# suhrig/arriba

Measured on AMD Instinct MI355X. Metric: chimeric reads/s end-to-end (BAM->fusions.tsv), synthetic, higher is better.
Workload: dtype int32

## Files before the change

### arriba_amd/_capi.py

```python
import ctypes
import os
from ctypes import POINTER, c_char_p, c_float, c_int, c_int32, c_size_t, c_uint8, c_uint16, c_uint32, c_uint64, c_void_p

LIB_DIR = os.path.join(os.path.dirname(os.path.abspath(__file__)), "lib")
FILTER_COUNT = 38
KERNEL_NAME_LENGTH = 48
FILTER_NAMES = [
    "", "duplicates", "inconsistently_clipped", "homopolymer", "read_through", "same_gene", "small_insert_size", "long_gap", "hairpin",
    "multimappers", "mismatches", "mismappers", "relative_support", "intronic", "non_coding_neighbors", "intragenic_exonic",
    "internal_tandem_duplication", "min_support", "known_fusions", "spliced", "blacklist", "end_to_end", "in_vitro", "merge_adjacent",
    "select_best", "marginal_read_through", "short_anchor", "no_coverage", "many_spliced", "no_genomic_support", "uninteresting_contigs",
    "viral_contigs", "top_expressed_viral_contigs", "low_coverage_viral_contigs", "genomic_support", "isoforms", "low_entropy", "homologs",
]


class FlatIndex(ctypes.Structure):
    _fields_ = [("n_contigs", c_uint32), ("contig_offset", POINTER(c_uint32)), ("n_keys", c_uint32), ("keys", POINTER(c_int32)),
                ("member_offset", POINTER(c_uint32)), ("n_members", c_uint32), ("members", POINTER(c_uint32))]


class AnnotationView(ctypes.Structure):
    _fields_ = [("n_genes", c_uint32), ("gene_contig", POINTER(c_uint16)), ("gene_start", POINTER(c_int32)), ("gene_end", POINTER(c_int32)),
                ("gene_bits", POINTER(c_uint8)), ("gene_exonic_length", POINTER(c_int32)),
                ("n_exons", c_uint32), ("exon_start", POINTER(c_int32)), ("exon_end", POINTER(c_int32)), ("exon_gene", POINTER(c_uint32)),
# ... 157 lines not shown
        "select_most_supported_breakpoints": (c_int, [ctx, POINTER(c_uint64)]),
        "recover_many_spliced": (c_int, [ctx, c_uint32, POINTER(c_uint64)]),
        "filter_in_vitro": (c_int, [ctx, c_float, POINTER(c_uint64)]),
        "filter_homologs": (c_int, [ctx, c_float, POINTER(c_uint64)]),
        "recover_isoforms": (c_int, [ctx, POINTER(c_uint64)]),
        "mark_genomic_support": (c_int, [ctx, POINTER(GenomicBreakpoint), c_uint32, c_int32, POINTER(c_uint64)]),
        "get_genomic_support": (c_int, [ctx, c_void_p, c_void_p]),
        "filter_no_genomic_support": (c_int, [ctx, POINTER(c_uint64)]),
        "recover_genomic_support": (c_int, [ctx, POINTER(c_uint64)]),
        "filter_blacklisted_ranges": (c_int, [ctx, POINTER(RangeRule), c_uint32, c_float, c_int32, POINTER(c_uint64)]),
        "recover_known_fusions": (c_int, [ctx, POINTER(RangeRule), c_uint32, c_int32, POINTER(c_uint64)]),
        "assign_confidence": (c_int, [ctx, c_void_p]),
        "recover_both_spliced": (c_int, [ctx, c_uint32, c_float, c_int32, c_uint32, POINTER(c_uint64)]),
        "set_owned_candidates": (c_int, [ctx, c_void_p, c_uint64]),
        "copy_multimapper_flags": (c_int, [ctx, c_void_p]),
        "multimappers_begin": (c_int, [ctx, c_void_p, POINTER(c_uint64)]),
        "multimappers_partial_best": (c_int, [ctx, c_void_p]),
        "multimappers_resolve": (c_int, [ctx, c_void_p, c_void_p, POINTER(c_uint64)]),
        "multimappers_recount": (c_int, [ctx, c_void_p, c_void_p]),
        "multimappers_finish": (c_int, [ctx, c_void_p, POINTER(c_uint64)]),
        "set_candidate_state": (c_int, [ctx, c_void_p, c_void_p, c_void_p, c_void_p]),
        "estimate_expected_fusions": (c_int, [ctx, c_uint64, c_void_p]),
        "get_evalues": (c_int, [ctx, c_void_p]),
        "filter_candidate_predicates": (c_int, [ctx, c_void_p]),
        "filter_relative_support": (c_int, [ctx, POINTER(c_uint64)]),
        "host_alloc": (c_void_p, [c_size_t]),
        "host_free": (None, [c_void_p]),
        "ingest_begin": (c_int, [ctx, POINTER(IngestConfig)]),
        "ingest_push": (c_int, [ctx, c_void_p, c_size_t]),
        "ingest_push_bgzf": (c_int, [ctx, c_void_p, c_size_t, POINTER(BgzfBlock), c_uint32, c_size_t]),
        "ingest_sam_targets": (c_int, [ctx, c_void_p, c_void_p, c_uint32]),
        "ingest_push_sam": (c_int, [ctx, c_void_p, c_size_t, c_uint64]),
        "sam_transcode": (c_int, [ctx, c_void_p, c_size_t, c_void_p, c_void_p, c_uint32, c_void_p, c_size_t, POINTER(c_uint64), POINTER(c_uint64), POINTER(c_uint64)]),
        "ingest_finish": (c_int, [ctx, POINTER(IngestResult)]),
        "shard_export_size": (c_int, [ctx, POINTER(c_uint64)]),
        "shard_export": (c_int, [ctx, c_void_p, c_uint64]),
        "shard_merge": (c_int, [ctx, c_void_p, c_uint64, c_uint32, POINTER(IngestResult)]),
        "mismapper_jobs": (c_int, [ctx, POINTER(c_uint64)]),
        "mismapper_verdicts": (c_int, [ctx, c_int32, c_uint32, c_uint32, c_void_p]),
        "filter_mismappers_apply": (c_int, [ctx, c_void_p, POINTER(c_uint64), POINTER(c_uint64)]),
        "get_viral_read_counts": (c_int, [ctx, c_void_p]),
        "get_coverage": (c_int, [ctx, c_void_p, c_void_p, c_void_p]),
        "detect_strandedness": (c_int, [ctx, POINTER(c_int)]),
        "get_read_lengths": (c_int, [ctx, c_uint64, c_uint64, c_void_p, c_void_p]),
        "gather_rows_begin": (c_int, [ctx, c_void_p, c_uint64, POINTER(c_uint64), POINTER(c_uint64), POINTER(c_uint64)]),
        "gather_rows_copy": (c_int, [ctx, POINTER(BatchRows)]),
        "set_profiling": (c_int, [ctx, c_int]),
        "debug_fail_allocation_in_finish": (None, [c_int]),
        "keep_batch_buffers": (c_int, [ctx, c_int]),
        "get_kernel_profile": (c_int, [ctx, c_void_p, c_void_p, c_void_p, c_uint32, POINTER(c_uint32)]),
        "last_kernel_ms": (c_int, [ctx, POINTER(c_float)]),
        "last_kernel_bytes": (c_int, [ctx, POINTER(c_uint64)]),
    }
    for name, (restype, argtypes) in signatures.items():
        function = getattr(lib, prefix + name, None)
        if function is None:
            continue
        function.restype = restype
        function.argtypes = argtypes
        setattr(api, name, function)
    api.exported = sorted(name for name in signatures if hasattr(api, name))
    api.declared = sorted(signatures)
    return api


def bind_host_api(lib):
# ... 132 lines not shown
```

### arriba_amd/csrc/device/agpu_ingest.hip

```cpp
#include <hip/hip_runtime.h>
#include <algorithm>
#include <cstring>
#include <string>
#include <vector>
#include <rocprim/rocprim.hpp>
#include "agpu_context.hpp"
#include "ingest_core.hpp"
#include "device_utils.hpp"
#include "shard_host.hpp"
#include "crc32_core.hpp"
#include "inflate_fast_core.hpp"

using namespace agpu;
namespace agpu { extern thread_local bool g_inside_ingest_finish; }

namespace {

const int BLOCK = 256;
inline unsigned int grid_for(uint64_t n, int block = BLOCK) { return (unsigned int) ((n + block - 1) / block); }

enum { IC_ACTIVE = 0, IC_MAPPED_READS = 1, IC_MISSING_HI = 2, IC_BROKEN = 3, IC_MALFORMED = 4, IC_CHIMERIC = 5, IC_COLLISION = 6, IC_MISMATCH = 7, IC_UNSORTED = 8, IC_MAX_NAME = 9,
       IC_MAX_READ_LENGTH = 10, IC_STRAND_COUNT = 11, IC_STRAND_MATCHING = 12, IC_RUNS_UNSORTED = 13, IC_QNAME_COMMA = 14, IC_COUNT = 16 };

#define HIP_CHECK(call) do { hipError_t e_ = (call); if (e_ != hipSuccess) { set_last_error(std::string(#call) + ": " + hipGetErrorString(e_)); return AGPU_ERR_DEVICE; } } while (0)
// ... 329 lines not shown
	const FragmentSizes mine = sizes[ref];
	cigar_words[i] = mine.cigar_words; sequence_bytes[i] = mine.sequence_bytes; name_lengths[i] = mine.name_length;
	uint32_t differs = 0;
	if (i > 0 && qname_run != nullptr) differs = qname_run[ref >> 1] != qname_run[order[i - 1] >> 1];
	else if (i > 0) {
		const Rec a = load_record(in, group_first[ref >> 1]), b = load_record(in, group_first[order[i - 1] >> 1]);
		const uint32_t length = qname_length(a);
		differs = length != qname_length(b);
		for (uint32_t k = 0; k < length && !differs; ++k) differs = a.name[k] != b.name[k];
	}
	new_group[i] = differs;
}

__global__ void __launch_bounds__(BLOCK) AGPU_PACK_OCCUPANCY fragment_pack_kernel(IngestStream in, const uint32_t* group_first, const uint32_t* order, uint64_t n, const FragmentPlan* plain, const TandemPlan* itd,
                                                              const uint64_t* cigar_base, const uint64_t* sequence_base, const uint64_t* name_base, const uint32_t* group_id, PackTarget out, uint32_t* counters) {
	__shared__ uint32_t block_max;
	if (threadIdx.x == 0) block_max = 0;
	__syncthreads();
	const uint64_t i = blockIdx.x * (uint64_t) BLOCK + threadIdx.x;
	if (i == n) out.name_offset[n] = name_base[n];
	if (i < n) {
		const uint32_t ref = order[i], g = ref >> 1;
		const bool is_itd = ref & 1;
		Fragment3 f;
		normalize_plan(in, is_itd ? itd[g].plan : plain[g], is_itd ? &itd[g].tandem : nullptr, f);
		Rec storage;
		const FragmentName name = name_of(in, group_first, ref, storage);
		atomicMax(&block_max, write_fragment(in, f, name, i, cigar_base[i], sequence_base[i], name_base[i], group_id[i], out));
	}
	__syncthreads();
	if (threadIdx.x == 0 && block_max) atomicMax(&counters[IC_MAX_READ_LENGTH], block_max);
}

template <bool INFLATED> __global__ void __launch_bounds__(256) bgzf_crc_kernel(const uint8_t* raw, const agpu_bgzf_block* blocks, uint32_t n_blocks, const Crc32Tables* tables, unsigned int* mismatches) {
	__shared__ uint32_t slice[4][256];
	__shared__ uint32_t join[2][4][256];
	__shared__ uint32_t staged[4][CRC32_WAVE_LANES * (CRC32_ROUND_WORDS + 1)];
	for (uint32_t k = threadIdx.x; k < 4 * 256; k += 256) ((uint32_t*) slice)[k] = ((const uint32_t*) tables->slice)[k];
	for (uint32_t k = threadIdx.x; k < 2 * 4 * 256; k += 256) ((uint32_t*) join)[k] = ((const uint32_t*) tables->join)[k];
	const uint32_t wave = threadIdx.x / CRC32_WAVE_LANES, lane = threadIdx.x % CRC32_WAVE_LANES, b = blockIdx.x * 4 + wave;
	agpu_bgzf_block block;
	block.crc32 = 0; block.payload_size = 0; block.raw_offset = 0; block.payload_offset = 0;
	if (b < n_blocks) block = blocks[b];
	if (INFLATED) { block.raw_offset = block.stream_offset; block.payload_offset = 0; block.payload_size = block.isize; }
	const bool checked = b < n_blocks && block.crc32 != 0 && block.payload_size <= CRC32_VIRTUAL;
	const uint8_t* payload = raw + block.raw_offset + block.payload_offset;
	const uint32_t n = block.payload_size;
	uint32_t* mine = staged[wave];
	uint32_t c = 0;
	const bool by_chunks = checked && n >= 4;
	const uint32_t first_word = by_chunks ? (CRC32_VIRTUAL - n) / 4 : CRC32_VIRTUAL / 4;
	for (uint32_t round = 0; round < CRC32_WAVE_CHUNK / 4 / CRC32_ROUND_WORDS; ++round) {
		__syncthreads();
		for (uint32_t item = lane; item < CRC32_WAVE_LANES * CRC32_ROUND_WORDS; item += CRC32_WAVE_LANES) {
			const uint32_t chunk = item / CRC32_ROUND_WORDS, j = item % CRC32_ROUND_WORDS, w = chunk * (CRC32_WAVE_CHUNK / 4) + round * CRC32_ROUND_WORDS + j;
			mine[chunk * (CRC32_ROUND_WORDS + 1) + j] = w >= first_word ? crc32_virtual_word(payload, n, w) : 0u;
		}
		__syncthreads();
		for (uint32_t j = 0; j < CRC32_ROUND_WORDS; ++j) c = crc32_raw_step(slice, c, mine[lane * (CRC32_ROUND_WORDS + 1) + j]);
	}
	__syncthreads();
	mine[lane] = c;
	__syncthreads();
	if (lane % 8 == 0) { for (uint32_t i = 1; i < 8; ++i) c = crc32_apply(join[0], c) ^ mine[lane + i]; }
	__syncthreads();
	if (lane % 8 == 0) mine[lane] = c;
	__syncthreads();
	if (lane == 0 && checked) {
		for (uint32_t g = 1; g < 8; ++g) c = crc32_apply(join[1], c) ^ mine[8 * g];
		c ^= 0xFFFFFFFFu;
		if (n < 4) c = crc32_of_sliced(slice, payload, n);
		if (c != block.crc32) atomicAdd(mismatches, 1u);
	}
}

__global__ void shard_rebase_kernel(uint32_t* out, const uint32_t* in, uint64_t n, uint32_t base, const uint8_t* n_aln, uint32_t slot) {
	const uint64_t i = (uint64_t) blockIdx.x * blockDim.x + threadIdx.x;
	if (i < n) out[i] = in[i] + ((slot >= 3 || slot < n_aln[i]) ? base : 0u);
}
__global__ void shard_rebase_names_kernel(uint64_t* out, const uint64_t* in, uint64_t n, uint64_t base) {
	const uint64_t i = (uint64_t) blockIdx.x * blockDim.x + threadIdx.x;
	if (i < n) out[i] = in[i] + base;
}
__global__ void shard_add_coverage_kernel(uint32_t* windows, uint8_t* starts, uint8_t* ends, const uint32_t* part_windows, const uint8_t* part_starts, const uint8_t* part_ends, uint64_t n) {
	const uint64_t i = (uint64_t) blockIdx.x * blockDim.x + threadIdx.x;
	if (i < n) { windows[i] += part_windows[i]; starts[i] |= part_starts[i]; ends[i] |= part_ends[i]; }
}
__global__ void shard_add_counts_kernel(unsigned long long* counts, const unsigned long long* part, uint32_t n) {
	const uint32_t i = blockIdx.x * blockDim.x + threadIdx.x;
	if (i < n) counts[i] += part[i];
}

__global__ void packed_name_length_kernel(const uint64_t* name_offset, uint64_t n, uint32_t* longest) {
	const uint64_t i = blockIdx.x * (uint64_t) BLOCK + threadIdx.x;
	if (i < n) atomicMax(longest, (uint32_t) (name_offset[i + 1] - name_offset[i]));
}
__global__ void packed_name_chunk_kernel(const char* names, const uint64_t* name_offset, const uint32_t* order, uint64_t n, uint32_t chunk, uint64_t* keys) {
	const uint64_t i = blockIdx.x * (uint64_t) BLOCK + threadIdx.x;
	if (i >= n) return;
	const uint32_t row = order[i]; const uint64_t begin = name_offset[row]; const uint32_t length = (uint32_t) (name_offset[row + 1] - begin);
	uint64_t key = 0;
	for (uint32_t k = 0; k < 8; ++k) { const uint32_t at = 8 * chunk + k; key = key << 8 | (at < length ? (uint8_t) names[begin + at] : 0u); }
	keys[i] = key;
}
__global__ void packed_name_neighbours_kernel(const char* names, const uint64_t* name_offset, const uint32_t* order, uint64_t n, uint32_t* new_group, uint32_t* equal_names) {
	const uint64_t i = blockIdx.x * (uint64_t) BLOCK + threadIdx.x;
// ... 336 lines not shown

}

int agpu::ingest_grow_stream(agpu_ctx* ctx, uint64_t needed) { return grow_stream(ctx, needed); }
int agpu::ingest_piece_pushed(agpu_ctx* ctx) {
	TRY(wait_for_previous_push(ctx));
	++ctx->ingest_pushes;
	return windows_after_push(ctx);
}

bool agpu::release_ingest_buffers(agpu_ctx* ctx) {
	bool released = ctx->ingest_stream.ptr != nullptr;
	ctx->ingest_stream.release(); for (int k = 0; k < AGPU_PIECE_SLOTS; ++k) ctx->ingest_raw[k].release();
	if (!ctx->ingest_part_of_sample) ctx->coverage_windows32.release();
	static const char* const temporary[] = { "ingest.record_offset", "ingest.keys", "ingest.keys_sorted", "ingest.record_bits", "ingest.sorted_records", "ingest.head", "ingest.group_start", "ingest.first_flags", "ingest.stream_rank", "ingest.group_first", "ingest.group_begin", "ingest.group_count", "ingest.plain_plans", "ingest.itd_plans",
		"ingest.valid", "ingest.sizes", "ingest.refs", "ingest.order", "ingest.order_keys", "ingest.order_keys_sorted", "ingest.cigar_words", "ingest.sequence_bytes", "ingest.name_lengths", "ingest.new_group", "ingest.cigar_base",
		"ingest.sequence_base", "ingest.name_base", "ingest.group_id", "ingest.qname_differs", "ingest.qname_run", "ingest.run_keys", "ingest.run_keys_sorted", "ingest.window_rocprim", "ingest.segment_first", "ingest.segment_end", "ingest.segment_end_before", "ingest.segment_count", "ingest.segment_base", "ingest.segment_mismatch", "ingest.rocprim", "ingest.coverage_summed", "ingest.hit_index",
		"sam.wave_count", "sam.wave_base", "sam.line_start", "sam.record_size", "sam.record_offset", "sam.rocprim", "sam.tool_text", "sam.tool_records" };
	for (size_t k = 0; k < sizeof(temporary) / sizeof(temporary[0]); ++k) { DeviceBuffer& buffer = ctx->scratch(temporary[k]); if (buffer.ptr != nullptr) released = true; buffer.release(); }
	return released;
}

extern "C" {

void* agpu_host_alloc(size_t bytes) {
	void* pointer = nullptr;
	if (hipHostMalloc(&pointer, bytes ? bytes : 16, hipHostMallocDefault) != hipSuccess) { set_last_error("hipHostMalloc failed"); return nullptr; }
	return pointer;
}
void agpu_host_free(void* pointer) { if (pointer) (void) hipHostFree(pointer); }

static int gather_rows_prepare(agpu_ctx* ctx, const uint32_t* fragments, uint64_t n, uint64_t* pool_sizes);

int agpu_ingest_begin(agpu_ctx* ctx, const agpu_ingest_config* config) {
	if (!ctx || !config) { set_last_error("null argument"); return AGPU_ERR_INVALID; }
	if (!ctx->have_annotation || !ctx->have_genome) { set_last_error("annotation and genome must be uploaded before the ingest"); return AGPU_ERR_INVALID; }
	if (config->n_contigs != ctx->genome.n_contigs) { set_last_error("the genome view on the device does not hold the contigs of the BAM header (upload it after the header was parsed)"); return AGPU_ERR_INVALID; }
	HIP_CHECK(hipSetDevice(ctx->device));
	hipStream_t s = ctx->stream;
	{ std::lock_guard<std::mutex> lock(ctx->profile_mutex); ctx->failed_launch.clear(); }
	if (!ctx->piece_stream) {
		int least = 0, greatest = 0;
		HIP_CHECK(hipDeviceGetStreamPriorityRange(&least, &greatest));
		const char* priorities = getenv("ARRIBA_STREAM_PRIORITIES");
		const bool pieces_first = priorities == nullptr || strcmp(priorities, "stages") != 0;
		HIP_CHECK(hipStreamCreateWithPriority(&ctx->piece_stream, hipStreamNonBlocking, pieces_first ? greatest : (least + greatest) / 2));
		HIP_CHECK(hipStreamCreateWithPriority(&ctx->piece_stream2, hipStreamNonBlocking, pieces_first ? greatest : (least + greatest) / 2));
		for (int k = 0; k < AGPU_PIECE_SLOTS; ++k) { HIP_CHECK(hipEventCreateWithFlags(&ctx->piece_copied[k], hipEventDisableTiming | hipEventBlockingSync));  HIP_CHECK(hipEventCreateWithFlags(&ctx->piece_ready[k], hipEventDisableTiming)); HIP_CHECK(hipEventCreateWithFlags(&ctx->piece_done[k], hipEventDisableTiming)); }
	}
	if (config->host_buffers > AGPU_PIECE_SLOTS) { set_last_error("agpu_ingest_config.host_buffers: at most 4"); return AGPU_ERR_INVALID; }
	ctx->ingest_host_buffers = config->host_buffers < 2 ? 2 : config->host_buffers;
	ctx->ingest_n_targets = config->n_targets; ctx->ingest_first_record = config->first_record_offset; ctx->ingest_stream_size = 0; ctx->ingest_pushes = 0; ctx->ingest_deflated_pieces = false; ctx->ingest_sam = false;
	{ const char* knob = getenv("ARRIBA_VERIFY_CRC"); ctx->ingest_verify_crc = !(knob != nullptr && knob[0] == '0'); }
	ALLOC(ctx->scratch("ingest.crc_mismatches"), 8);
	if (ctx->ingest_verify_crc && ctx->scratch("ingest.crc_tables").ptr == nullptr) {
		ALLOC(ctx->scratch("ingest.crc_tables"), sizeof(Crc32Tables));
		static Crc32Tables tables; static bool made = false;
		if (!made) { crc32_make_tables(tables); made = true; }
		HIP_CHECK(hipMemcpy(ctx->scratch("ingest.crc_tables").ptr, &tables, sizeof(tables), hipMemcpyHostToDevice));
	}
	HIP_CHECK(hipMemsetAsync(ctx->scratch("ingest.crc_mismatches").ptr, 0, 8, s));
	ctx->ingest_external_duplicate_marking = config->external_duplicate_marking; ctx->ingest_max_itd_length = config->max_itd_length; ctx->ingest_part_of_sample = config->part_of_sample != 0;
	ALLOC(ctx->ingest_tid_to_contig, std::max<size_t>(config->n_targets, 1) * 4);
	if (config->n_targets) HIP_CHECK(hipMemcpyAsync(ctx->ingest_tid_to_contig.ptr, config->tid_to_contig, (size_t) config->n_targets * 4, hipMemcpyHostToDevice, s));
	ctx->host_coverage_window_offset.assign(config->coverage_window_offset, config->coverage_window_offset + config->n_contigs + 1);
	const uint64_t windows = ctx->host_coverage_window_offset.back();
	ALLOC(ctx->coverage_window_offset, ((size_t) config->n_contigs + 1) * 8); ALLOC(ctx->coverage_windows32, std::max<uint64_t>(coverage_difference_slots(windows, config->n_contigs), 1) * 4); ALLOC(ctx->coverage_windows, std::max<uint64_t>(windows, 1) * 2);
	ALLOC(ctx->coverage_fragment_starts, std::max<uint64_t>(windows, 1)); ALLOC(ctx->coverage_fragment_ends, std::max<uint64_t>(windows, 1));
	HIP_CHECK(hipMemcpyAsync(ctx->coverage_window_offset.ptr, config->coverage_window_offset, ((size_t) config->n_contigs + 1) * 8, hipMemcpyHostToDevice, s));
	HIP_CHECK(hipMemsetAsync(ctx->coverage_windows32.ptr, 0, std::max<uint64_t>(coverage_difference_slots(windows, config->n_contigs), 1) * 4, s));
	HIP_CHECK(hipMemsetAsync(ctx->coverage_fragment_starts.ptr, 0, std::max<uint64_t>(windows, 1), s));
	HIP_CHECK(hipMemsetAsync(ctx->coverage_fragment_ends.ptr, 0, std::max<uint64_t>(windows, 1), s));
	ALLOC(ctx->ingest_viral_counts, std::max<size_t>(config->n_contigs, 1) * 8);
	HIP_CHECK(hipMemsetAsync(ctx->ingest_viral_counts.ptr, 0, std::max<size_t>(config->n_contigs, 1) * 8, s));
	if (config->stream_size_hint > 0) TRY(grow_stream(ctx, config->stream_size_hint));
	{
		IngestProgress& p = ctx->ingest_progress;
		for (size_t k = 0; k < p.windows.size(); ++k) p.events.push_back(p.windows[k].readback);
		p.windows.clear();
		const char* knob = getenv("ARRIBA_INGEST_WINDOWS");
		p.on = !ctx->ingest_part_of_sample && !(knob != nullptr && knob[0] == '0' && knob[1] == 0);
		g_window_bytes = 512u << 20; g_window_margin = 1u << 20;
		if (knob != nullptr && strchr(knob, ',') != nullptr) { g_window_bytes = strtoull(knob, nullptr, 10); g_window_margin = std::max<uint64_t>(strtoull(strchr(knob, ',') + 1, nullptr, 10), 1); }
		p.abandoned = false; p.touched = false; p.next_slot = 0; p.window_bytes = 0; p.segments_done = 0; p.records = 0; p.active = 0; p.heads = 0; p.groups_done = 0; p.windows_made = 0; p.size_hint = config->stream_size_hint;
		if (p.on) {
			if (!p.work) {
				int least = 0, greatest = 0;
				HIP_CHECK(hipDeviceGetStreamPriorityRange(&least, &greatest));
				HIP_CHECK(hipStreamCreateWithPriority(&p.work, hipStreamNonBlocking, least));
				HIP_CHECK(hipHostMalloc((void**) &p.host_words, INGEST_WINDOW_RING * INGEST_WINDOW_WORDS * 4, hipHostMallocDefault));
			}
			ALLOC(ctx->scratch("ingest.window_words"), INGEST_WINDOW_RING * INGEST_WINDOW_WORDS * 4); ALLOC(ctx->scratch("ingest.window_state"), 16); ALLOC(ctx->scratch("ingest.counters"), IC_COUNT * 4);
			HIP_CHECK(hipMemsetAsync(ctx->scratch("ingest.window_state").ptr, 0, 16, s));
// ... 36 lines not shown
		if (deflated) ALLOC(ctx->scratch("ingest.inflate_spill"), 2 * 65536);
		HIP_CHECK(hipStreamWaitEvent(s, ctx->piece_done[slot], 0));
		HIP_CHECK(hipMemcpyAsync(ctx->ingest_raw[slot].ptr, raw, raw_size, hipMemcpyHostToDevice, s));
		HIP_CHECK(hipMemcpyAsync(ctx->ingest_blocks[slot].ptr, blocks, (size_t) n_blocks * sizeof(agpu_bgzf_block), hipMemcpyHostToDevice, s));
		HIP_CHECK(hipEventRecord(ctx->piece_copied[slot], s));
		HIP_CHECK(hipStreamWaitEvent(pieces, ctx->piece_copied[slot], 0));
		if (deflated) {
			ctx->ingest_deflated_pieces = true;
			uint8_t* target = ctx->ingest_stream.as<uint8_t>() + ctx->ingest_stream_size;
			unsigned int* failures = ctx->scratch("ingest.crc_mismatches").as<unsigned int>() + 1;
			static const char* way = getenv("ARRIBA_INFLATE");
			if (way != nullptr && strcmp(way, "wave") == 0) {
				KernelTimer timer(ctx, "bgzf_inflate_kernel", (uint64_t) raw_size + stream_bytes, pieces);
				bgzf_inflate_kernel<<<n_blocks, 64, 0, pieces>>>(ctx->ingest_raw[slot].as<uint8_t>(), ctx->ingest_blocks[slot].as<agpu_bgzf_block>(), target, ctx->scratch("ingest.inflate_spill").as<uint8_t>(), nullptr, failures);
			} else {
				DeviceBuffer& notes = ctx->scratch(set ? "ingest.inflate_notes2" : "ingest.inflate_notes"); DeviceBuffer& note_count = ctx->scratch(set ? "ingest.inflate_note_count2" : "ingest.inflate_note_count"); DeviceBuffer& status = ctx->scratch(set ? "ingest.inflate_status2" : "ingest.inflate_status");
				if ((size_t) n_blocks * INFLATE_MATCH_CAPACITY * 8 > notes.capacity || (size_t) n_blocks * 4 > status.capacity) {
					HIP_CHECK(hipStreamSynchronize(pieces));
					ALLOC(notes, (size_t) n_blocks * INFLATE_MATCH_CAPACITY * 8); ALLOC(note_count, (size_t) n_blocks * 4); ALLOC(status, (size_t) n_blocks * 4);
				}
				const int lanes = way != nullptr && atoi(way) > 0 ? atoi(way) : 20;
				{ KernelTimer timer(ctx, "bgzf_inflate_tokens_kernel", (uint64_t) raw_size + stream_bytes, pieces);
				  #define TOKENS(LANES) bgzf_inflate_tokens_kernel<LANES><<<(n_blocks + LANES - 1) / LANES, LANES, 0, pieces>>>(ctx->ingest_raw[slot].as<uint8_t>(), ctx->ingest_blocks[slot].as<agpu_bgzf_block>(), n_blocks, target, \
				  	ctx->scratch("ingest.inflate_spill").as<uint8_t>(), notes.as<unsigned long long>(), note_count.as<uint32_t>(), status.as<int>(), failures)
				  if (lanes == 16) TOKENS(16); else if (lanes == 24) TOKENS(24); else TOKENS(20);
				  #undef TOKENS
				}
				bgzf_inflate_kernel<<<n_blocks, 64, 0, pieces>>>(ctx->ingest_raw[slot].as<uint8_t>(), ctx->ingest_blocks[slot].as<agpu_bgzf_block>(), target, ctx->scratch("ingest.inflate_spill").as<uint8_t>(), status.as<int>(), failures);
				{ KernelTimer timer(ctx, "bgzf_inflate_resolve_kernel", (uint64_t) stream_bytes, pieces);
				  bgzf_inflate_resolve_kernel<<<(n_blocks + BLOCK / 64 - 1) / (BLOCK / 64), BLOCK, 0, pieces>>>(ctx->ingest_blocks[slot].as<agpu_bgzf_block>(), n_blocks, target, ctx->scratch("ingest.inflate_spill").as<uint8_t>(),
				  	notes.as<unsigned long long>(), note_count.as<uint32_t>(), status.as<int>()); }
			}
		}
		else { KernelTimer timer(ctx, "bgzf_unwrap_kernel", (uint64_t) raw_size + stream_bytes, pieces);
		  bgzf_unwrap_kernel<<<n_blocks, BLOCK, 0, pieces>>>(ctx->ingest_raw[slot].as<uint8_t>(), ctx->ingest_blocks[slot].as<agpu_bgzf_block>(), ctx->ingest_stream.as<uint8_t>() + ctx->ingest_stream_size); }
		const uint64_t piece_stream_offset = ctx->ingest_stream_size;
		ctx->ingest_stream_size += stream_bytes;
		if (ctx->ingest_pushes > 0) HIP_CHECK(hipStreamWaitEvent(pieces, ctx->piece_ready[(ctx->ingest_pushes - 1) % AGPU_PIECE_SLOTS], 0));
		HIP_CHECK(hipEventRecord(ctx->piece_ready[slot], pieces));
		if (ctx->ingest_verify_crc) {
			KernelTimer timer(ctx, "bgzf_crc_kernel", deflated ? stream_bytes : raw_size, pieces);
			if (deflated) bgzf_crc_kernel<true><<<(n_blocks + 3) / 4, 256, 0, pieces>>>(ctx->ingest_stream.as<uint8_t>() + piece_stream_offset, ctx->ingest_blocks[slot].as<agpu_bgzf_block>(), n_blocks, ctx->scratch("ingest.crc_tables").as<Crc32Tables>(), ctx->scratch("ingest.crc_mismatches").as<unsigned int>());
			else bgzf_crc_kernel<false><<<(n_blocks + 3) / 4, 256, 0, pieces>>>(ctx->ingest_raw[slot].as<uint8_t>(), ctx->ingest_blocks[slot].as<agpu_bgzf_block>(), n_blocks, ctx->scratch("ingest.crc_tables").as<Crc32Tables>(), ctx->scratch("ingest.crc_mismatches").as<unsigned int>());
		}
		HIP_CHECK(hipEventRecord(ctx->piece_done[slot], pieces));
	} else { HIP_CHECK(hipEventRecord(ctx->piece_copied[slot], s)); HIP_CHECK(hipEventRecord(ctx->piece_ready[slot], s)); }
	TRY(wait_for_previous_push(ctx));
	++ctx->ingest_pushes;
	return windows_after_push(ctx);
}

int agpu_ingest_finish(agpu_ctx* ctx, agpu_ingest_result* result) {
	if (!ctx || !ctx->ingest_active) { set_last_error("agpu_ingest_begin must run first"); return AGPU_ERR_INVALID; }
	HIP_CHECK(hipSetDevice(ctx->device));
	hipStream_t s = ctx->stream;
	ctx->ingest_active = false;
	struct Finishing { agpu_ctx* ctx; explicit Finishing(agpu_ctx* c) : ctx(c) { ctx->ingest_finishing = true; g_inside_ingest_finish = true; } ~Finishing() { ctx->ingest_finishing = false; g_inside_ingest_finish = false; } } finishing(ctx);
	const uint64_t size = ctx->ingest_stream_size, base = ctx->ingest_first_record;
	if (base > size) { set_last_error("failed to read SAM header"); return AGPU_ERR_INVALID; }
	if (agpu::debug_finish_runs_out_of_memory(ctx)) { set_last_error("hipMalloc failed (the buffers of the batch; asked for by agpu_debug_exhaust_memory_in_finish)"); return AGPU_ERR_NO_MEMORY; }
	if (!ctx->keeps_batch_buffers) take_sample_buffers(ctx);
	HIP_CHECK(hipStreamSynchronize(ctx->piece_stream)); HIP_CHECK(hipStreamSynchronize(ctx->piece_stream2));
	if (ctx->ingest_verify_crc || ctx->ingest_deflated_pieces) {
		unsigned int mismatches[2] = { 0, 0 };
		HIP_CHECK(hipMemcpyAsync(mismatches, ctx->scratch("ingest.crc_mismatches").ptr, 8, hipMemcpyDeviceToHost, s));
		HIP_CHECK(hipStreamSynchronize(s));
		if (mismatches[1] > 0 || (ctx->ingest_verify_crc && mismatches[0] > 0)) { set_last_error("failed to load alignments"); return AGPU_ERR_INVALID; }
	}
	if (ctx->ingest_sam) {
		const int verdict = agpu::sam_ingest_verdict(ctx);
		if (verdict != AGPU_OK) { if (ctx->ingest_progress.work) HIP_CHECK(hipStreamSynchronize(ctx->ingest_progress.work));  return verdict; }
	}
	DeviceBuffer& counters = ctx->scratch("ingest.counters"); DeviceBuffer& rocprim_scratch = ctx->scratch("ingest.rocprim");
	ALLOC(counters, IC_COUNT * 4);
	uint32_t* device_counters = counters.as<uint32_t>();
	uint32_t host_counters[IC_COUNT];
	auto read_counters = [&]() -> int { HIP_CHECK(hipMemcpyAsync(host_counters, counters.ptr, IC_COUNT * 4, hipMemcpyDeviceToHost, s)); HIP_CHECK(hipStreamSynchronize(s)); return AGPU_OK; };
	(void) hipEventRecord(ctx->event_start, s);

	IngestProgress& progress = ctx->ingest_progress;
	bool streamed = false;
	if (progress.on) {
// ... 742 lines not shown
```

### arriba_amd/csrc/device/crc32_core.hpp

```cpp
#ifndef AGPU_CRC32_CORE_HPP
#define AGPU_CRC32_CORE_HPP 1

#include "views.hpp"

namespace agpu {

const uint32_t CRC32_POLYNOMIAL = 0xEDB88320u;

AGPU_HD uint32_t crc32_table_entry(uint32_t i) {
	uint32_t c = i;
	for (int k = 0; k < 8; ++k) c = (c & 1u) ? (c >> 1) ^ CRC32_POLYNOMIAL : c >> 1;
	return c;
}
AGPU_HD uint32_t crc32_of(const uint32_t* table, const uint8_t* bytes, size_t n) {
	uint32_t c = 0xFFFFFFFFu;
	for (size_t i = 0; i < n; ++i) c = table[(c ^ bytes[i]) & 0xFFu] ^ (c >> 8);
	return c ^ 0xFFFFFFFFu;
}
AGPU_HD uint32_t gf2_matrix_times(const uint32_t* matrix, uint32_t vector) {
	uint32_t sum = 0;
	for (int k = 0; vector != 0; vector >>= 1, ++k) if (vector & 1u) sum ^= matrix[k];
	return sum;
}
AGPU_HD void gf2_matrix_square(uint32_t* square, const uint32_t* matrix) { for (int k = 0; k < 32; ++k) square[k] = gf2_matrix_times(matrix, matrix[k]); }
// ... 47 lines not shown
	return word;
}
inline uint32_t crc32_fold_chunks(const Crc32Tables& t, const uint32_t* chunk ) {
	uint32_t group[8];
	for (uint32_t g = 0; g < 8; ++g) { uint32_t c = chunk[8 * g]; for (uint32_t i = 1; i < 8; ++i) c = crc32_apply(t.join[0], c) ^ chunk[8 * g + i]; group[g] = c; }
	uint32_t c = group[0];
	for (uint32_t g = 1; g < 8; ++g) c = crc32_apply(t.join[1], c) ^ group[g];
	return c ^ 0xFFFFFFFFu;
}
inline void crc32_make_tables(Crc32Tables& t) {
	for (uint32_t i = 0; i < 256; ++i) t.slice[0][i] = crc32_table_entry(i);
	for (int k = 1; k < 4; ++k) for (uint32_t i = 0; i < 256; ++i) t.slice[k][i] = (t.slice[k - 1][i] >> 8) ^ t.slice[0][t.slice[k - 1][i] & 0xFFu];
	uint32_t even[32], odd[32];
	odd[0] = CRC32_POLYNOMIAL;
	uint32_t row = 1;
	for (int k = 1; k < 32; ++k) { odd[k] = row; row <<= 1; }
	gf2_matrix_square(even, odd); gf2_matrix_square(odd, even);
	gf2_matrix_square(t.advance[0], odd);
	for (int k = 1; k < CRC32_ADVANCE_POWERS; ++k) gf2_matrix_square(t.advance[k], t.advance[k - 1]);
	for (int j = 0; j < 2; ++j)
		for (uint32_t b = 0; b < 4; ++b) for (uint32_t v = 0; v < 256; ++v) t.join[j][b][v] = gf2_matrix_times(t.advance[j == 0 ? 10 : 13], v << (8 * b));
}
AGPU_HD uint32_t crc32_of_sliced(const uint32_t (*slice)[256], const uint8_t* bytes, size_t n) {
	uint32_t c = 0xFFFFFFFFu;
	size_t i = 0;
	for (; i + 4 <= n; i += 4) {
		uint32_t word; __builtin_memcpy(&word, bytes + i, 4);
		c ^= word;
		c = slice[3][c & 0xFFu] ^ slice[2][(c >> 8) & 0xFFu] ^ slice[1][(c >> 16) & 0xFFu] ^ slice[0][c >> 24];
	}
	for (; i < n; ++i) c = slice[0][(c ^ bytes[i]) & 0xFFu] ^ (c >> 8);
	return c ^ 0xFFFFFFFFu;
}
AGPU_HD uint32_t crc32_joined_with(const uint32_t (*advance)[32], uint32_t crc_a, uint32_t crc_b, uint32_t length_b) {
	for (int k = 0; length_b != 0; length_b >>= 1, ++k) if (length_b & 1u) crc_a = gf2_matrix_times(advance[k], crc_a);
	return crc_a ^ crc_b;
}

}

#endif
```

### include/arriba_gpu.h

```cpp
#ifndef ARRIBA_GPU_H
#define ARRIBA_GPU_H 1

#include <stddef.h>
#include <stdint.h>

#ifdef __cplusplus
extern "C" {
#endif

#define AGPU_API_VERSION 1

#define AGPU_OK 0
#define AGPU_ERR_INVALID (-1)
#define AGPU_ERR_DEVICE (-2)
#define AGPU_ERR_CAPACITY (-3)
#define AGPU_ERR_NO_DEVICE (-4)
#define AGPU_ERR_NO_MEMORY (-5)

#define AGPU_FILTER_COUNT 38

#define AGPU_ABIT_STRAND 1u
#define AGPU_ABIT_FIRST_IN_PAIR 2u
#define AGPU_ABIT_SUPPLEMENTARY 4u
#define AGPU_ABIT_EXONIC 8u
// ... 124 lines not shown
	const uint32_t* tid_to_contig;
	uint64_t first_record_offset;
	uint64_t stream_size_hint;
	uint32_t n_contigs;
	const uint64_t* coverage_window_offset;
	uint8_t external_duplicate_marking;
	uint32_t max_itd_length;
	uint8_t part_of_sample;
	uint8_t host_buffers;
} agpu_ingest_config;
typedef struct { uint64_t raw_offset; uint32_t payload_offset, payload_size; uint64_t stream_offset; uint32_t crc32; uint32_t isize; uint32_t skip; uint32_t keep; } agpu_bgzf_block;
typedef struct {
	uint64_t records;
	uint64_t fragments;
	uint64_t mapped_reads;
	uint64_t malformed_count;
	uint64_t missing_hi_tag;
	uint8_t no_chimeric_reads;
	uint8_t names_were_sorted;
	uint16_t windows;
	uint8_t reserved[4];
	uint64_t stream_bytes;
} agpu_ingest_result;
void* agpu_host_alloc(size_t bytes);
void agpu_host_free(void* pointer);
int agpu_keep_batch_buffers(agpu_ctx* ctx, int on);
int agpu_ingest_begin(agpu_ctx* ctx, const agpu_ingest_config* config);
int agpu_ingest_push(agpu_ctx* ctx, const void* bytes, size_t size);
int agpu_ingest_push_bgzf(agpu_ctx* ctx, const void* raw, size_t raw_size, const agpu_bgzf_block* blocks, uint32_t n_blocks, size_t stream_bytes);
int agpu_ingest_finish(agpu_ctx* ctx, agpu_ingest_result* result);
int agpu_ingest_sam_targets(agpu_ctx* ctx, const char* names, const uint32_t* name_offset, uint32_t n_targets);
int agpu_ingest_push_sam(agpu_ctx* ctx, const void* text, size_t size, uint64_t first_line_number);
int agpu_sam_transcode(agpu_ctx* ctx, const void* text, size_t size, const char* names, const uint32_t* name_offset, uint32_t n_targets, void* out, size_t capacity, uint64_t* out_bytes, uint64_t* n_records, uint64_t* bad_line);
int agpu_get_viral_read_counts(agpu_ctx* ctx, uint64_t* counts );
int agpu_get_coverage(agpu_ctx* ctx, uint16_t* coverage, uint8_t* fragment_starts, uint8_t* fragment_ends);
int agpu_detect_strandedness(agpu_ctx* ctx, int* strandedness);
int agpu_get_read_lengths(agpu_ctx* ctx, uint64_t first, uint64_t count, uint32_t* mate1, uint32_t* mate2);
typedef struct {
	uint64_t n;
	uint8_t* n_aln; uint8_t* fbits; uint32_t* group;
	uint16_t* contig[3]; int32_t* start[3]; int32_t* end[3]; uint8_t* abits[3]; uint32_t* cigar_offset[3]; uint16_t* cigar_count[3];
	uint64_t cigar_pool_size; uint32_t* cigar_pool;
	uint32_t* seq_offset[2]; uint32_t* seq_length[2];
	uint64_t seq_pool_size; uint8_t* seq_pool;
	uint32_t* name_offset;
	uint64_t names_size; char* names;
} agpu_batch_rows;
int agpu_gather_rows_begin(agpu_ctx* ctx, const uint32_t* fragments , uint64_t n, uint64_t* cigar_pool_size, uint64_t* seq_pool_size, uint64_t* names_size);
int agpu_gather_rows_copy(agpu_ctx* ctx, agpu_batch_rows* rows);

int agpu_shard_export_size(agpu_ctx* ctx, uint64_t* bytes);
int agpu_shard_export(agpu_ctx* ctx, void* block, uint64_t capacity);
int agpu_shard_merge(agpu_ctx* ctx, const void* blocks, uint64_t stride, uint32_t n_parts, agpu_ingest_result* result );

int agpu_shard_merge_rccl(agpu_ctx* ctx, void* nccl_comm, uint32_t n_ranks, agpu_ingest_result* result);
int agpu_filter_mismappers_rccl(agpu_ctx* ctx, void* nccl_comm, int32_t max_mate_gap, uint32_t rank, uint32_t n_ranks, uint64_t* remaining, uint64_t* discarded_reads);
#define AGPU_RCCL_ID_BYTES 128
enum { AGPU_REDUCE_MAX_INT64 = 0, AGPU_REDUCE_MIN_INT64 = 1, AGPU_REDUCE_SUM_INT64 = 2, AGPU_REDUCE_MAX_BYTES = 3, AGPU_REDUCE_SUM_UINT32 = 4  };
int agpu_rccl_unique_id(uint8_t* id );
int agpu_rccl_join(agpu_ctx* ctx, const uint8_t* id, uint32_t rank, uint32_t n_ranks, void** nccl_comm);
int agpu_rccl_leave(void* nccl_comm);
int agpu_rccl_all_gather_host(agpu_ctx* ctx, void* nccl_comm, uint32_t n_ranks, const void* mine, void* all, uint64_t bytes);
int agpu_rccl_all_reduce_host(agpu_ctx* ctx, void* nccl_comm, void* values, uint64_t count, int kind);
int agpu_rccl_all_gather_device(agpu_ctx* ctx, void* nccl_comm, const void* mine, void* all , uint64_t bytes);
int agpu_rccl_all_reduce_device(agpu_ctx* ctx, void* nccl_comm, void* values, uint64_t count, int kind);
int agpu_scratch_buffer(agpu_ctx* ctx, const char* name, uint64_t bytes, void** pointer);
// ... 155 lines not shown
```

Before: 60.82 million.

## Fuse BGZF stored-block unwrap with CRC check in one wave-per-block kernel

Stored (uncompressed) BGZF pieces are now copied and CRC-checked in a single kernel that reads each payload once. The kernel uses one 64-lane wave per workgroup in a grid-stride loop over blocks, with 16-byte vector loads, software-prefetched rounds and wave-level barriers instead of __syncthreads. Join tables are read from global memory rather than staged in LDS. This removes a second full pass over the raw bytes and the block-wide syncs. It also adds a standalone agpu_bgzf_unwrap API and an environment switch that restores the two-kernel path.

```diff
diff --git a/arriba_amd/_capi.py b/arriba_amd/_capi.py
--- a/arriba_amd/_capi.py
+++ b/arriba_amd/_capi.py
@@ -213,6 +213,7 @@
         "ingest_sam_targets": (c_int, [ctx, c_void_p, c_void_p, c_uint32]),
         "ingest_push_sam": (c_int, [ctx, c_void_p, c_size_t, c_uint64]),
         "sam_transcode": (c_int, [ctx, c_void_p, c_size_t, c_void_p, c_void_p, c_uint32, c_void_p, c_size_t, POINTER(c_uint64), POINTER(c_uint64), POINTER(c_uint64)]),
+        "bgzf_unwrap": (c_int, [ctx, c_void_p, c_size_t, POINTER(BgzfBlock), c_uint32, c_void_p, c_size_t, POINTER(c_uint32)]),
         "ingest_finish": (c_int, [ctx, POINTER(IngestResult)]),
         "shard_export_size": (c_int, [ctx, POINTER(c_uint64)]),
         "shard_export": (c_int, [ctx, c_void_p, c_uint64]),
diff --git a/arriba_amd/csrc/device/agpu_ingest.hip b/arriba_amd/csrc/device/agpu_ingest.hip
--- a/arriba_amd/csrc/device/agpu_ingest.hip
+++ b/arriba_amd/csrc/device/agpu_ingest.hip
@@ -385,46 +385,77 @@
 	if (threadIdx.x == 0 && block_max) atomicMax(&counters[IC_MAX_READ_LENGTH], block_max);
 }
 
-template <bool INFLATED> __global__ void __launch_bounds__(256) bgzf_crc_kernel(const uint8_t* raw, const agpu_bgzf_block* blocks, uint32_t n_blocks, const Crc32Tables* tables, unsigned int* mismatches) {
+const uint32_t CRC32_STAGE_STRIDE = CRC32_WIDE_ROUND_WORDS + 1, CONTAINER_WORKGROUPS = 4096;
+__device__ __forceinline__ Crc32Unit load_unit(const uint8_t* p) { Crc32Unit u; __builtin_memcpy(&u, p, CRC32_UNIT); return u; }
+__device__ __forceinline__ void store_unit(uint8_t* p, const Crc32Unit& u) { __builtin_memcpy(p, &u, CRC32_UNIT); }
+template <bool STORE> __device__ __forceinline__ void container_block(const uint8_t* payload, uint32_t n, uint32_t expected, bool checked, uint8_t* target, const uint32_t (*slice)[256], uint32_t* staged, const Crc32Tables* tables, unsigned int* mismatches) {
+	const uint32_t lane = threadIdx.x;
+	if (n < 4 || n > CRC32_VIRTUAL) {
+		if (STORE) for (uint32_t i = lane; i < n; i += CRC32_WAVE_LANES) target[i] = payload[i];
+		if (lane == 0 && checked && n < 4 && (crc32_of_sliced(slice, payload, n) != expected)) atomicAdd(mismatches, 1u);
+		return;
+	}
+	const Crc32Unit first = load_unit(payload);
+	const Crc32Unit head = crc32_head_unit(first, n);
+	const uint32_t head_bytes = (CRC32_UNIT - (CRC32_VIRTUAL - n) % CRC32_UNIT) % CRC32_UNIT;
+	if (STORE && lane < head_bytes) target[lane] = (uint8_t) ((lane < 4 ? first.w[0] : lane < 8 ? first.w[1] : lane < 12 ? first.w[2] : first.w[3]) >> (8 * (lane % 4)));
+	const int32_t mine = crc32_unit_start(n, lane / 8, 0, lane % 8);
+	Crc32Unit next[8];
+	#pragma unroll
+	for (uint32_t k = 0; k < 8; ++k) { const int32_t m = mine + (int32_t) (k * 8 * CRC32_WAVE_CHUNK); next[k] = load_unit(payload + (m > 0 ? m : 0)); }
+	uint32_t c = 0;
+	for (uint32_t round = 0; round < CRC32_WIDE_ROUNDS; ++round) {
+		Crc32Unit now[8];
+		#pragma unroll
+		for (uint32_t k = 0; k < 8; ++k) now[k] = next[k];
+		if (round + 1 < CRC32_WIDE_ROUNDS) {
+			#pragma unroll
+			for (uint32_t k = 0; k < 8; ++k) { const int32_t m = mine + (int32_t) (k * 8 * CRC32_WAVE_CHUNK + (round + 1) * 4 * CRC32_WIDE_ROUND_WORDS); next[k] = load_unit(payload + (m > 0 ? m : 0)); }
+		}
+		#pragma unroll
+		for (uint32_t k = 0; k < 8; ++k) {
+			const int32_t m = mine + (int32_t) (k * 8 * CRC32_WAVE_CHUNK + round * 4 * CRC32_WIDE_ROUND_WORDS);
+			if (STORE && m >= 0) store_unit(target + m, now[k]);
+			const Crc32Unit unit = crc32_virtual_unit(now[k], head, m);
+			uint32_t* at = staged + (8 * k + lane / 8) * CRC32_STAGE_STRIDE + 4 * (lane % 8);
+			at[0] = unit.w[0]; at[1] = unit.w[1]; at[2] = unit.w[2]; at[3] = unit.w[3];
+		}
+		__builtin_amdgcn_fence(__ATOMIC_RELEASE, "wavefront"); __builtin_amdgcn_wave_barrier(); __builtin_amdgcn_fence(__ATOMIC_ACQUIRE, "wavefront");
+		#pragma unroll
+		for (uint32_t j = 0; j < CRC32_WIDE_ROUND_WORDS; ++j) c = crc32_raw_step(slice, c, staged[lane * CRC32_STAGE_STRIDE + j]);
+		__builtin_amdgcn_fence(__ATOMIC_RELEASE, "wavefront"); __builtin_amdgcn_wave_barrier();
+	}
+	if (!checked) return;
+	uint32_t others[7];
+	#pragma unroll
+	for (uint32_t i = 1; i < 8; ++i) others[i - 1] = __shfl(c, (lane + i) % CRC32_WAVE_LANES);
+	if (lane % 8 == 0) { for (uint32_t i = 1; i < 8; ++i) c = crc32_apply(tables->join[0], c) ^ others[i - 1]; }
+	#pragma unroll
+	for (uint32_t g = 1; g < 8; ++g) others[g - 1] = __shfl(c, 8 * g);
+	if (lane == 0) {
+		for (uint32_t g = 1; g < 8; ++g) c = crc32_apply(tables->join[1], c) ^ others[g - 1];
+		if ((c ^ 0xFFFFFFFFu) != expected) atomicAdd(mismatches, 1u);
+	}
+}
+template <bool INFLATED, bool STORE> __device__ __forceinline__ void container_pass(const uint8_t* raw, const agpu_bgzf_block* blocks, uint32_t n_blocks, const Crc32Tables* tables, unsigned int* mismatches, uint8_t* stream) {
 	__shared__ uint32_t slice[4][256];
-	__shared__ uint32_t join[2][4][256];
-	__shared__ uint32_t staged[4][CRC32_WAVE_LANES * (CRC32_ROUND_WORDS + 1)];
-	for (uint32_t k = threadIdx.x; k < 4 * 256; k += 256) ((uint32_t*) slice)[k] = ((const uint32_t*) tables->slice)[k];
-	for (uint32_t k = threadIdx.x; k < 2 * 4 * 256; k += 256) ((uint32_t*) join)[k] = ((const uint32_t*) tables->join)[k];
-	const uint32_t wave = threadIdx.x / CRC32_WAVE_LANES, lane = threadIdx.x % CRC32_WAVE_LANES, b = blockIdx.x * 4 + wave;
-	agpu_bgzf_block block;
-	block.crc32 = 0; block.payload_size = 0; block.raw_offset = 0; block.payload_offset = 0;
-	if (b < n_blocks) block = blocks[b];
-	if (INFLATED) { block.raw_offset = block.stream_offset; block.payload_offset = 0; block.payload_size = block.isize; }
-	const bool checked = b < n_blocks && block.crc32 != 0 && block.payload_size <= CRC32_VIRTUAL;
-	const uint8_t* payload = raw + block.raw_offset + block.payload_offset;
-	const uint32_t n = block.payload_size;
-	uint32_t* mine = staged[wave];
-	uint32_t c = 0;
-	const bool by_chunks = checked && n >= 4;
-	const uint32_t first_word = by_chunks ? (CRC32_VIRTUAL - n) / 4 : CRC32_VIRTUAL / 4;
-	for (uint32_t round = 0; round < CRC32_WAVE_CHUNK / 4 / CRC32_ROUND_WORDS; ++round) {
-		__syncthreads();
-		for (uint32_t item = lane; item < CRC32_WAVE_LANES * CRC32_ROUND_WORDS; item += CRC32_WAVE_LANES) {
-			const uint32_t chunk = item / CRC32_ROUND_WORDS, j = item % CRC32_ROUND_WORDS, w = chunk * (CRC32_WAVE_CHUNK / 4) + round * CRC32_ROUND_WORDS + j;
-			mine[chunk * (CRC32_ROUND_WORDS + 1) + j] = w >= first_word ? crc32_virtual_word(payload, n, w) : 0u;
-		}
-		__syncthreads();
-		for (uint32_t j = 0; j < CRC32_ROUND_WORDS; ++j) c = crc32_raw_step(slice, c, mine[lane * (CRC32_ROUND_WORDS + 1) + j]);
-	}
-	__syncthreads();
-	mine[lane] = c;
-	__syncthreads();
-	if (lane % 8 == 0) { for (uint32_t i = 1; i < 8; ++i) c = crc32_apply(join[0], c) ^ mine[lane + i]; }
-	__syncthreads();
-	if (lane % 8 == 0) mine[lane] = c;
-	__syncthreads();
-	if (lane == 0 && checked) {
-		for (uint32_t g = 1; g < 8; ++g) c = crc32_apply(join[1], c) ^ mine[8 * g];
-		c ^= 0xFFFFFFFFu;
-		if (n < 4) c = crc32_of_sliced(slice, payload, n);
-		if (c != block.crc32) atomicAdd(mismatches, 1u);
-	}
+	__shared__ uint32_t staged[CRC32_WAVE_LANES * CRC32_STAGE_STRIDE];
+	for (uint32_t k = threadIdx.x; k < 4 * 256; k += CRC32_WAVE_LANES) ((uint32_t*) slice)[k] = ((const uint32_t*) tables->slice)[k];
+	__builtin_amdgcn_fence(__ATOMIC_RELEASE, "wavefront"); __builtin_amdgcn_wave_barrier(); __builtin_amdgcn_fence(__ATOMIC_ACQUIRE, "wavefront");
+	for (uint32_t b = blockIdx.x; b < n_blocks; b += gridDim.x) {
+		const agpu_bgzf_block block = blocks[b];
+		const uint8_t* payload = INFLATED ? raw + block.stream_offset : raw + block.raw_offset + block.payload_offset;
+		const uint32_t n = INFLATED ? block.isize : block.payload_size;
+		const bool checked = block.crc32 != 0 && n <= CRC32_VIRTUAL;
+		if (!STORE && !checked) continue;
+		container_block<STORE>(payload, n, block.crc32, checked, STORE ? stream + block.stream_offset : nullptr, slice, staged, tables, mismatches);
+	}
+}
+template <bool INFLATED> __global__ void __launch_bounds__(64) bgzf_crc_kernel(const uint8_t* raw, const agpu_bgzf_block* blocks, uint32_t n_blocks, const Crc32Tables* tables, unsigned int* mismatches) {
+	container_pass<INFLATED, false>(raw, blocks, n_blocks, tables, mismatches, nullptr);
+}
+__global__ void __launch_bounds__(64) bgzf_unwrap_crc_kernel(const uint8_t* raw, const agpu_bgzf_block* blocks, uint32_t n_blocks, const Crc32Tables* tables, unsigned int* mismatches, uint8_t* stream) {
+	container_pass<false, true>(raw, blocks, n_blocks, tables, mismatches, stream);
 }
 
 __global__ void shard_rebase_kernel(uint32_t* out, const uint32_t* in, uint64_t n, uint32_t base, const uint8_t* n_aln, uint32_t slot) {
@@ -827,6 +858,33 @@
 
 static int gather_rows_prepare(agpu_ctx* ctx, const uint32_t* fragments, uint64_t n, uint64_t* pool_sizes);
 
+static int prepare_crc(agpu_ctx* ctx) {
+	{ const char* knob = getenv("ARRIBA_VERIFY_CRC"); ctx->ingest_verify_crc = !(knob != nullptr && knob[0] == '0'); }
+	ALLOC(ctx->scratch("ingest.crc_mismatches"), 8);
+	if (ctx->ingest_verify_crc && ctx->scratch("ingest.crc_tables").ptr == nullptr) {
+		ALLOC(ctx->scratch("ingest.crc_tables"), sizeof(Crc32Tables));
+		static Crc32Tables tables; static bool made = false;
+		if (!made) { crc32_make_tables(tables); made = true; }
+		HIP_CHECK(hipMemcpy(ctx->scratch("ingest.crc_tables").ptr, &tables, sizeof(tables), hipMemcpyHostToDevice));
+	}
+	return AGPU_OK;
+}
+static void launch_stored_piece(agpu_ctx* ctx, hipStream_t on, const uint8_t* raw, size_t raw_size, const agpu_bgzf_block* blocks, uint32_t n_blocks, uint8_t* target, size_t stream_bytes) {
+	static const bool two_kernels = getenv("ARRIBA_CONTAINER_PASS") != nullptr && strcmp(getenv("ARRIBA_CONTAINER_PASS"), "two") == 0;
+	if (ctx->ingest_verify_crc && two_kernels) {
+		{ KernelTimer timer(ctx, "bgzf_unwrap_kernel", (uint64_t) raw_size + stream_bytes, on);
+		  bgzf_unwrap_kernel<<<n_blocks, BLOCK, 0, on>>>(raw, blocks, target); }
+		KernelTimer timer(ctx, "bgzf_crc_kernel", raw_size, on);
+		bgzf_crc_kernel<false><<<std::min(n_blocks, CONTAINER_WORKGROUPS), 64, 0, on>>>(raw, blocks, n_blocks, ctx->scratch("ingest.crc_tables").as<Crc32Tables>(), ctx->scratch("ingest.crc_mismatches").as<unsigned int>());
+	} else if (ctx->ingest_verify_crc) {
+		KernelTimer timer(ctx, "bgzf_unwrap_crc_kernel", (uint64_t) raw_size + stream_bytes, on);
+		bgzf_unwrap_crc_kernel<<<std::min(n_blocks, CONTAINER_WORKGROUPS), 64, 0, on>>>(raw, blocks, n_blocks, ctx->scratch("ingest.crc_tables").as<Crc32Tables>(), ctx->scratch("ingest.crc_mismatches").as<unsigned int>(), target);
+	} else {
+		KernelTimer timer(ctx, "bgzf_unwrap_kernel", (uint64_t) raw_size + stream_bytes, on);
+		bgzf_unwrap_kernel<<<n_blocks, BLOCK, 0, on>>>(raw, blocks, target);
+	}
+}
+
 int agpu_ingest_begin(agpu_ctx* ctx, const agpu_ingest_config* config) {
 	if (!ctx || !config) { set_last_error("null argument"); return AGPU_ERR_INVALID; }
 	if (!ctx->have_annotation || !ctx->have_genome) { set_last_error("annotation and genome must be uploaded before the ingest"); return AGPU_ERR_INVALID; }
@@ -846,14 +904,7 @@
 	if (config->host_buffers > AGPU_PIECE_SLOTS) { set_last_error("agpu_ingest_config.host_buffers: at most 4"); return AGPU_ERR_INVALID; }
 	ctx->ingest_host_buffers = config->host_buffers < 2 ? 2 : config->host_buffers;
 	ctx->ingest_n_targets = config->n_targets; ctx->ingest_first_record = config->first_record_offset; ctx->ingest_stream_size = 0; ctx->ingest_pushes = 0; ctx->ingest_deflated_pieces = false; ctx->ingest_sam = false;
-	{ const char* knob = getenv("ARRIBA_VERIFY_CRC"); ctx->ingest_verify_crc = !(knob != nullptr && knob[0] == '0'); }
-	ALLOC(ctx->scratch("ingest.crc_mismatches"), 8);
-	if (ctx->ingest_verify_crc && ctx->scratch("ingest.crc_tables").ptr == nullptr) {
-		ALLOC(ctx->scratch("ingest.crc_tables"), sizeof(Crc32Tables));
-		static Crc32Tables tables; static bool made = false;
-		if (!made) { crc32_make_tables(tables); made = true; }
-		HIP_CHECK(hipMemcpy(ctx->scratch("ingest.crc_tables").ptr, &tables, sizeof(tables), hipMemcpyHostToDevice));
-	}
+	TRY(prepare_crc(ctx));
 	HIP_CHECK(hipMemsetAsync(ctx->scratch("ingest.crc_mismatches").ptr, 0, 8, s));
 	ctx->ingest_external_duplicate_marking = config->external_duplicate_marking; ctx->ingest_max_itd_length = config->max_itd_length; ctx->ingest_part_of_sample = config->part_of_sample != 0;
 	ALLOC(ctx->ingest_tid_to_contig, std::max<size_t>(config->n_targets, 1) * 4);
@@ -956,22 +1007,51 @@
 				  	notes.as<unsigned long long>(), note_count.as<uint32_t>(), status.as<int>()); }
 			}
 		}
-		else { KernelTimer timer(ctx, "bgzf_unwrap_kernel", (uint64_t) raw_size + stream_bytes, pieces);
-		  bgzf_unwrap_kernel<<<n_blocks, BLOCK, 0, pieces>>>(ctx->ingest_raw[slot].as<uint8_t>(), ctx->ingest_blocks[slot].as<agpu_bgzf_block>(), ctx->ingest_stream.as<uint8_t>() + ctx->ingest_stream_size); }
+		else launch_stored_piece(ctx, pieces, ctx->ingest_raw[slot].as<uint8_t>(), raw_size, ctx->ingest_blocks[slot].as<agpu_bgzf_block>(), n_blocks, ctx->ingest_stream.as<uint8_t>() + ctx->ingest_stream_size, stream_bytes);
 		const uint64_t piece_stream_offset = ctx->ingest_stream_size;
 		ctx->ingest_stream_size += stream_bytes;
 		if (ctx->ingest_pushes > 0) HIP_CHECK(hipStreamWaitEvent(pieces, ctx->piece_ready[(ctx->ingest_pushes - 1) % AGPU_PIECE_SLOTS], 0));
 		HIP_CHECK(hipEventRecord(ctx->piece_ready[slot], pieces));
-		if (ctx->ingest_verify_crc) {
-			KernelTimer timer(ctx, "bgzf_crc_kernel", deflated ? stream_bytes : raw_size, pieces);
-			if (deflated) bgzf_crc_kernel<true><<<(n_blocks + 3) / 4, 256, 0, pieces>>>(ctx->ingest_stream.as<uint8_t>() + piece_stream_offset, ctx->ingest_blocks[slot].as<agpu_bgzf_block>(), n_blocks, ctx->scratch("ingest.crc_tables").as<Crc32Tables>(), ctx->scratch("ingest.crc_mismatches").as<unsigned int>());
-			else bgzf_crc_kernel<false><<<(n_blocks + 3) / 4, 256, 0, pieces>>>(ctx->ingest_raw[slot].as<uint8_t>(), ctx->ingest_blocks[slot].as<agpu_bgzf_block>(), n_blocks, ctx->scratch("ingest.crc_tables").as<Crc32Tables>(), ctx->scratch("ingest.crc_mismatches").as<unsigned int>());
+		if (ctx->ingest_verify_crc && deflated) {
+			KernelTimer timer(ctx, "bgzf_crc_kernel", stream_bytes, pieces);
+			bgzf_crc_kernel<true><<<std::min(n_blocks, CONTAINER_WORKGROUPS), 64, 0, pieces>>>(ctx->ingest_stream.as<uint8_t>() + piece_stream_offset, ctx->ingest_blocks[slot].as<agpu_bgzf_block>(), n_blocks, ctx->scratch("ingest.crc_tables").as<Crc32Tables>(), ctx->scratch("ingest.crc_mismatches").as<unsigned int>());
 		}
 		HIP_CHECK(hipEventRecord(ctx->piece_done[slot], pieces));
 	} else { HIP_CHECK(hipEventRecord(ctx->piece_copied[slot], s)); HIP_CHECK(hipEventRecord(ctx->piece_ready[slot], s)); }
 	TRY(wait_for_previous_push(ctx));
 	++ctx->ingest_pushes;
 	return windows_after_push(ctx);
+}
+
+int agpu_bgzf_unwrap(agpu_ctx* ctx, const void* raw, size_t raw_size, const agpu_bgzf_block* blocks, uint32_t n_blocks, void* stream_out, size_t stream_bytes, uint32_t* crc_mismatches) {
+	if (!ctx || (!raw && raw_size > 0) || (!blocks && n_blocks > 0) || (!stream_out && stream_bytes > 0) || !crc_mismatches) { set_last_error("null argument"); return AGPU_ERR_INVALID; }
+	if (ctx->ingest_active) { set_last_error("agpu_bgzf_unwrap: an ingest is under way on this context"); return AGPU_ERR_INVALID; }
+	*crc_mismatches = 0;
+	for (uint32_t b = 0; b < n_blocks; ++b) {
+		const agpu_bgzf_block& block = blocks[b];
+		if (block.isize != 0) { set_last_error("agpu_bgzf_unwrap: stored blocks only"); return AGPU_ERR_INVALID; }
+		if (block.raw_offset > raw_size || block.payload_offset > raw_size - block.raw_offset || block.payload_size > raw_size - block.raw_offset - block.payload_offset) { set_last_error("agpu_bgzf_unwrap: a payload lies outside the piece"); return AGPU_ERR_INVALID; }
+		if (block.stream_offset > stream_bytes || block.payload_size > stream_bytes - block.stream_offset) { set_last_error("agpu_bgzf_unwrap: a target lies outside the stream"); return AGPU_ERR_INVALID; }
+	}
+	HIP_CHECK(hipSetDevice(ctx->device));
+	hipStream_t s = ctx->stream;
+	TRY(prepare_crc(ctx));
+	DeviceBuffer& device_raw = ctx->scratch("bgzf.tool_raw"); DeviceBuffer& device_blocks = ctx->scratch("bgzf.tool_blocks"); DeviceBuffer& device_stream = ctx->scratch("bgzf.tool_stream");
+	ALLOC(device_raw, raw_size + 256); ALLOC(device_blocks, (size_t) std::max(n_blocks, 1u) * sizeof(agpu_bgzf_block)); ALLOC(device_stream, stream_bytes + 64);
+	HIP_CHECK(hipMemsetAsync(ctx->scratch("ingest.crc_mismatches").ptr, 0, 8, s));
+	HIP_CHECK(hipMemsetAsync(device_stream.ptr, 0, stream_bytes + 64, s));
+	if (n_blocks > 0 && raw_size > 0) {
+		HIP_CHECK(hipMemcpyAsync(device_raw.ptr, raw, raw_size, hipMemcpyHostToDevice, s));
+		HIP_CHECK(hipMemcpyAsync(device_blocks.ptr, blocks, (size_t) n_blocks * sizeof(agpu_bgzf_block), hipMemcpyHostToDevice, s));
+		launch_stored_piece(ctx, s, device_raw.as<uint8_t>(), raw_size, device_blocks.as<agpu_bgzf_block>(), n_blocks, device_stream.as<uint8_t>(), stream_bytes);
+		HIP_CHECK(hipGetLastError());
+	}
+	unsigned int mismatches[2] = { 0, 0 };
+	HIP_CHECK(hipMemcpyAsync(mismatches, ctx->scratch("ingest.crc_mismatches").ptr, 8, hipMemcpyDeviceToHost, s));
+	if (stream_bytes > 0) HIP_CHECK(hipMemcpyAsync(stream_out, device_stream.ptr, stream_bytes, hipMemcpyDeviceToHost, s));
+	HIP_CHECK(hipStreamSynchronize(s));
+	*crc_mismatches = mismatches[0];
+	return AGPU_OK;
 }
 
 int agpu_ingest_finish(agpu_ctx* ctx, agpu_ingest_result* result) {
diff --git a/arriba_amd/csrc/device/crc32_core.hpp b/arriba_amd/csrc/device/crc32_core.hpp
--- a/arriba_amd/csrc/device/crc32_core.hpp
+++ b/arriba_amd/csrc/device/crc32_core.hpp
@@ -103,6 +103,29 @@
 	for (; i < n; ++i) c = slice[0][(c ^ bytes[i]) & 0xFFu] ^ (c >> 8);
 	return c ^ 0xFFFFFFFFu;
 }
+const uint32_t CRC32_UNIT = 16, CRC32_WIDE_ROUND_WORDS = 32, CRC32_WIDE_ROUNDS = CRC32_WAVE_CHUNK / 4 / CRC32_WIDE_ROUND_WORDS;
+struct Crc32Unit { uint32_t w[4]; };
+AGPU_HD Crc32Unit crc32_head_unit(Crc32Unit first, uint32_t n) {
+	const uint32_t s = (CRC32_VIRTUAL - n) % CRC32_UNIT;
+	first.w[0] ^= 0xFFFFFFFFu;
+	uint64_t low = first.w[0] | (uint64_t) first.w[1] << 32, high = first.w[2] | (uint64_t) first.w[3] << 32;
+	if (s >= 8) { high = low << (8 * (s - 8)); low = 0; }
+	else if (s > 0) { high = high << (8 * s) | low >> (64 - 8 * s); low <<= 8 * s; }
+	Crc32Unit head;
+	head.w[0] = (uint32_t) low; head.w[1] = (uint32_t) (low >> 32); head.w[2] = (uint32_t) high; head.w[3] = (uint32_t) (high >> 32);
+	return head;
+}
+AGPU_HD Crc32Unit crc32_virtual_unit(Crc32Unit loaded, const Crc32Unit& head, int32_t m) {
+	const bool zero = m <= -(int32_t) CRC32_UNIT, front = m < 0;
+	Crc32Unit unit;
+	for (int k = 0; k < 4; ++k) unit.w[k] = zero ? 0u : front ? head.w[k] : loaded.w[k];
+	unit.w[0] ^= (uint32_t) m < 4u ? 0xFFFFFFFFu >> (8 * ((uint32_t) m & 3u)) : 0u;
+	return unit;
+}
+AGPU_HD int32_t crc32_unit_start(uint32_t n, uint32_t chunk, uint32_t round, uint32_t part) {
+	return (int32_t) (chunk * CRC32_WAVE_CHUNK + round * 4 * CRC32_WIDE_ROUND_WORDS + part * CRC32_UNIT) - (int32_t) (CRC32_VIRTUAL - n);
+}
+
 AGPU_HD uint32_t crc32_joined_with(const uint32_t (*advance)[32], uint32_t crc_a, uint32_t crc_b, uint32_t length_b) {
 	for (int k = 0; length_b != 0; length_b >>= 1, ++k) if (length_b & 1u) crc_a = gf2_matrix_times(advance[k], crc_a);
 	return crc_a ^ crc_b;
diff --git a/include/arriba_gpu.h b/include/arriba_gpu.h
--- a/include/arriba_gpu.h
+++ b/include/arriba_gpu.h
@@ -180,6 +180,7 @@
 int agpu_ingest_sam_targets(agpu_ctx* ctx, const char* names, const uint32_t* name_offset, uint32_t n_targets);
 int agpu_ingest_push_sam(agpu_ctx* ctx, const void* text, size_t size, uint64_t first_line_number);
 int agpu_sam_transcode(agpu_ctx* ctx, const void* text, size_t size, const char* names, const uint32_t* name_offset, uint32_t n_targets, void* out, size_t capacity, uint64_t* out_bytes, uint64_t* n_records, uint64_t* bad_line);
+int agpu_bgzf_unwrap(agpu_ctx* ctx, const void* raw, size_t raw_size, const agpu_bgzf_block* blocks, uint32_t n_blocks, void* stream_out, size_t stream_bytes, uint32_t* crc_mismatches);
 int agpu_get_viral_read_counts(agpu_ctx* ctx, uint64_t* counts );
 int agpu_get_coverage(agpu_ctx* ctx, uint16_t* coverage, uint8_t* fragment_starts, uint8_t* fragment_ends);
 int agpu_detect_strandedness(agpu_ctx* ctx, int* strandedness);
```

Measured after the change: 59.06 million. 2.9% lower.
